# ffreyer/MonteCarlo.jl

Hardware: AMD Instinct MI355X
Metric: DQMC sweeps/sec, 16x16 Hubbard beta=8 dtau=0.1; achieved % fp64 MFMA roofline (higher is better)
Workload: dtype f64

## Files before the change

### montecarlo.jl_amd/csrc/sweep_lu.hip

```cpp
#include "kernels.h"
#include <hip/hip_ext.h>
#include <cstdlib>

namespace dqmc {

typedef double d4 __attribute__((ext_vector_type(4)));

size_t sweep_lu_image_doubles() { return LU_STRIDE; }

__device__ __forceinline__ double readlane_d(double v, int lane)
{
    const unsigned long long u = (unsigned long long)__double_as_longlong(v);
    const unsigned lo = (unsigned)__builtin_amdgcn_readlane((int)(u & 0xffffffffull), lane);
    const unsigned hi = (unsigned)__builtin_amdgcn_readlane((int)(u >> 32), lane);
    return __longlong_as_double((long long)(((unsigned long long)hi << 32) | lo));
}
#define MFMA(a, b, c) __builtin_amdgcn_mfma_f64_16x16x4f64((a), (b), (c), 0, 0, 0)
#define DQMC_GLOBAL __attribute__((address_space(1)))
typedef const DQMC_GLOBAL double *gcdp;
typedef DQMC_GLOBAL double *gdp;
typedef double d2v __attribute__((ext_vector_type(2)));
typedef const DQMC_GLOBAL d2v *gcd2p;


constexpr int LU4_SPIN = 1 << 21;
template <int NB>
struct Lu4Smem {
    double2 aST[NB][64][64];
    double xs[NB][64];
    double strip[12][NB][2][64];
    double negv[64];
    int step[64];
    int sflag[12];
    unsigned acc16[4], neg16[4];
    int ndraw[4], exh[4];
    int abort;
};
__host__ __device__ constexpr int lu4_strip_idx(int I0, int r0, int I) { return I0 == 0 ? r0 * 2 + (I - 1) : 8 + r0; }

#define LU4_ORDER() asm volatile("" ::: "memory")

__device__ __forceinline__ int lu4_wait(int *flag, int *abortf)
{
    int v = 0;
    for (int it = 0; it < LU4_SPIN; ++it) {
        v = __builtin_amdgcn_readfirstlane(__hip_atomic_load(flag, __ATOMIC_RELAXED, __HIP_MEMORY_SCOPE_WORKGROUP));
        if (v) break;
        if ((it & 63) == 63 &&
            __builtin_amdgcn_readfirstlane(__hip_atomic_load(abortf, __ATOMIC_RELAXED, __HIP_MEMORY_SCOPE_WORKGROUP)))
            return -1;
        __builtin_amdgcn_s_sleep(1);
    }
    if (!v) {
        __hip_atomic_store(abortf, 1, __ATOMIC_RELAXED, __HIP_MEMORY_SCOPE_WORKGROUP);
        return -1;
    }
    LU4_ORDER();
    return v;
}
__device__ __forceinline__ double lu4_rcp(double r)
{
    double y = __builtin_amdgcn_rcp(r);
    double e = __builtin_fma(-r, y, 1.0);
    y = __builtin_fma(y, e, y);
    e = __builtin_fma(-r, y, 1.0);
    return __builtin_fma(y, e, y);
}

extern __shared__ __attribute__((aligned(16))) double lu4_lds[];
#ifdef LU4_STAMPS
__device__ long long *lu4_stamp_ptr = nullptr;
#define LU4_STAMP(idx)                                                                       \
    do {                                                                                     \
        if ((LU4_STAMPS != 2 || (idx) >= 320) && w == 0 && (threadIdx.x & 63) == 0 && lu4_stamp_ptr)            \
            lu4_stamp_ptr[(idx)] = (long long)__builtin_amdgcn_s_memtime();                  \
    } while (0)
#else
#define LU4_STAMP(idx) do { } while (0)
#endif
#ifdef LU4_STAMPS
#ifndef FL_STAMP_BID
#define FL_STAMP_BID 1200
#endif
#define FL_STAMP(k)                                                                                    \
    do {                                                                                               \
        if (bid == FL_STAMP_BID && threadIdx.x == 0 && lu4_stamp_ptr)                                 \
            lu4_stamp_ptr[480 + (k)] = (long long)__builtin_amdgcn_s_memtime();                       \
    } while (0)
#else
#define FL_STAMP(k) do { } while (0)
#endif
template <int NB, bool FULL, bool PRO, int J>
__device__ __noinline__ void lu4_wave(int n, const double *__restrict__ Gall, long strideG, int w, int site0,
                                      int nsites, double *__restrict__ img_all, const SweepConsts &sc,
                                      unsigned long long cbits_v, double uvec, int check_sign, int site0p,
                                      const double *__restrict__ imgp_all)
{
    Lu4Smem<NB> &sm = *reinterpret_cast<Lu4Smem<NB> *>(lu4_lds);
    const int lane = threadIdx.x & 63, g = lane >> 4, ci = lane & 15;
    const unsigned long long cbits =
        ((unsigned long long)(unsigned)__builtin_amdgcn_readfirstlane((int)(cbits_v >> 32)) << 32) |
        (unsigned)__builtin_amdgcn_readfirstlane((int)(cbits_v & 0xffffffffull));
    d4 S[NB][J + 1], ST[NB][J + 1];
#pragma unroll
    for (int b = 0; b < NB; ++b) {
        const gcdp G = (gcdp)(Gall + (long)(w * NB + b) * strideG + (long)site0 * n + site0);
#pragma unroll
        for (int I = 0; I <= J; ++I)
#pragma unroll
            for (int r = 0; r < 4; ++r) {
                const int rho = 16 * I + 4 * r + g, kap = 16 * J + ci;
                if (FULL) {
                    S[b][I][r] = G[rho + (long)n * kap];
                    ST[b][I][r] = G[kap + (long)n * rho];
                } else {
                    const bool ok = rho < nsites && kap < nsites;
                    const int rc = min(rho, nsites - 1), kc = min(kap, nsites - 1);
                    const double a = G[rc + (long)n * kc], c = G[kc + (long)n * rc];
                    S[b][I][r] = ok ? a : 0.0;
                    ST[b][I][r] = ok ? c : 0.0;
                }
            }
    }
    if (PRO) {
        LU4_STAMP(400 + 8 * J + 0);
        constexpr bool EARLY = (NB == 1) && (sizeof(Lu4Smem<NB>) + LU_STRIDE * sizeof(double) <= 150 * 1024);
        double *xtra = lu4_lds + (sizeof(Lu4Smem<NB>) + 15) / 16 * 2 + LU_STRIDE;
        double *Rl = EARLY ? reinterpret_cast<double *>(&sm.aST[0][31][0]) : reinterpret_cast<double *>(&sm.aST[0][0][0]);
        double *ttx = EARLY ? xtra : Rl + 64 * 66;
        double *tt0 = xtra + 1536;
        int *pflag = reinterpret_cast<int *>(xtra + 1536 + 1024);
        const int tid = threadIdx.x;
#pragma unroll 1
        for (int b = 0; b < NB; ++b) {
            const gcdp Gin = (gcdp)(Gall + (long)(w * NB + b) * strideG);
            const gcdp imgp = (gcdp)(imgp_all + (long)(w * NB + b) * LU_STRIDE);
            const int t = site0 + 16 * J + ci;
            d4 az[4];
#pragma unroll
            for (int Jb = 0; Jb < 4; ++Jb)
#pragma unroll
                for (int r = 0; r < 4; ++r) az[Jb][r] = Gin[t + (long)n * (site0p + 16 * Jb + 4 * r + g)];
            constexpr bool STAGE = sizeof(Lu4Smem<NB>) + LU_STRIDE * sizeof(double) <= 150 * 1024;
            auto r0_col = [&](int i) { return STAGE ? (i * 256 + tid) >> 5 : tid >> 2; };
            auto r0_row = [&](int i) { return STAGE ? 2 * ((i * 256 + tid) & 31) : (tid & 3) * 16 + 2 * i; };
            d2v r0v[8];
#pragma unroll
            for (int i = 0; i < 8; ++i)
                r0v[i] = *reinterpret_cast<gcd2p>(Gin + (long)n * (site0 + r0_col(i)) + site0p + r0_row(i));
            double *imgl = lu4_lds + (sizeof(Lu4Smem<NB>) + 15) / 16 * 2;
            double opU[STAGE ? 1 : 6][4], opL[STAGE ? 1 : 6][4], opP[STAGE ? 1 : 4][4], opQ[STAGE ? 1 : 4][4], xr[4][4];
            if (STAGE) {
                constexpr int NI = (LU_STRIDE / 2 + 255) / 256;
                const gcd2p src = reinterpret_cast<gcd2p>(imgp);
                d2v *dst = reinterpret_cast<d2v *>(imgl);
                d2v iv[NI];
#pragma unroll
                for (int i = 0; i < NI; ++i) iv[i] = src[min(tid + 256 * i, LU_STRIDE / 2 - 1)];
                __builtin_amdgcn_sched_barrier(0);
#pragma unroll
                for (int i = 0; i < NI; ++i) dst[min(tid + 256 * i, LU_STRIDE / 2 - 1)] = iv[i];
            } else {
#pragma unroll
                for (int pr = 0; pr < (STAGE ? 0 : 6); ++pr)
#pragma unroll
                    for (int q = 0; q < 4; ++q) {
                        opU[pr][q] = imgp[LU_OFF_U + pr * LU_TILE + q * 64 + lane];
                        opL[pr][q] = imgp[LU_OFF_L + pr * LU_TILE + q * 64 + lane];
                    }
#pragma unroll
                for (int Jb = 0; Jb < (STAGE ? 0 : 4); ++Jb)
#pragma unroll
                    for (int q = 0; q < 4; ++q) {
                        opP[Jb][q] = imgp[LU_OFF_PT + Jb * LU_TILE + q * 64 + lane];
                        opQ[Jb][q] = imgp[LU_OFF_Q + Jb * LU_TILE + q * 64 + lane];
                    }
            }
#pragma unroll
            for (int i = 0; i < 8; ++i) *reinterpret_cast<d2v *>(Rl + r0_col(i) * 66 + r0_row(i)) = r0v[i];
            if (STAGE) __syncthreads();
#pragma unroll
            for (int Jb = 0; Jb < 4; ++Jb)
#pragma unroll
                for (int q = 0; q < 4; ++q) xr[Jb][q] = STAGE ? imgl[LU_IMG + 16 * Jb + 4 * q + g] : imgp[LU_IMG + 16 * Jb + 4 * q + g];
#define PRO_U(pr, q) (STAGE ? imgl[LU_OFF_U + (pr) * LU_TILE + (q) * 64 + lane] : opU[STAGE ? 0 : (pr)][q])
#define PRO_L(pr, q) (STAGE ? imgl[LU_OFF_L + (pr) * LU_TILE + (q) * 64 + lane] : opL[STAGE ? 0 : (pr)][q])
#define PRO_P(jb, q) (STAGE ? imgl[LU_OFF_PT + (jb) * LU_TILE + (q) * 64 + lane] : opP[STAGE ? 0 : (jb)][q])
#define PRO_Q(jb, q) (STAGE ? imgl[LU_OFF_Q + (jb) * LU_TILE + (q) * 64 + lane] : opQ[STAGE ? 0 : (jb)][q])
            d4 xz[4], tt[4];
#if defined(LU4_STAMPS) && LU4_STAMPS != 2
            LU4_STAMP(400 + 8 * J + 1);
            asm volatile("s_waitcnt vmcnt(0)" ::: "memory");
            LU4_STAMP(400 + 8 * J + 2);
#endif
#pragma unroll
            for (int Jb = 0; Jb < 4; ++Jb) {
#pragma unroll
                for (int K = 0; K < Jb; ++K)
#pragma unroll
                    for (int q = 0; q < 4; ++q) az[Jb] = MFMA(PRO_U(lu_pair(K, Jb), q), xz[K][q], az[Jb]);
                d4 z = {0.0, 0.0, 0.0, 0.0};
#pragma unroll
                for (int q = 0; q < 4; ++q) z = MFMA(PRO_P(Jb, q), az[Jb][q], z);
#pragma unroll
                for (int r = 0; r < 4; ++r) xz[Jb][r] = z[r] * xr[Jb][r];
            }
#pragma unroll
            for (int Jb = 3; Jb >= 0; --Jb) {
                d4 a = {0.0, 0.0, 0.0, 0.0};
#pragma unroll
                for (int K = Jb + 1; K < 4; ++K)
#pragma unroll
                    for (int q = 0; q < 4; ++q) a = MFMA(PRO_L(lu_pair(Jb, K), q), tt[K][q], a);
#pragma unroll
                for (int r = 0; r < 4; ++r) a[r] = xz[Jb][r] + xr[Jb][r] * a[r];
                d4 o = {0.0, 0.0, 0.0, 0.0};
#pragma unroll
                for (int q = 0; q < 4; ++q) o = MFMA(PRO_Q(Jb, q), a[q], o);
                tt[Jb] = o;
            }
#undef PRO_U
#undef PRO_L
#undef PRO_P
#undef PRO_Q
            LU4_STAMP(400 + 8 * J + 3);
            if (EARLY) {
                double *dlt = ttx;
                if (J == 0) {
#pragma unroll
                    for (int K = 0; K < 4; ++K)
#pragma unroll
                        for (int q = 0; q < 4; ++q) tt0[(K * 4 + q) * 64 + lane] = tt[K][q];
                    LU4_ORDER();
                    __hip_atomic_store(&pflag[0], 1, __ATOMIC_RELAXED, __HIP_MEMORY_SCOPE_WORKGROUP);
#pragma unroll
                    for (int K = 0; K < 4; ++K)
#pragma unroll
                        for (int q = 0; q < 4; ++q) {
                            const int sk = 16 * K + 4 * q + g;
                            ST[b][0] = MFMA(Rl[ci * 66 + sk], tt[K][q], ST[b][0]);
                            S[b][0] = MFMA(tt[K][q], Rl[ci * 66 + sk], S[b][0]);
                        }
                } else {
#pragma unroll
                    for (int K = 0; K < 4; ++K)
#pragma unroll
                        for (int q = 0; q < 4; ++q) {
                            const int sk = 16 * K + 4 * q + g;
#pragma unroll
                            for (int I = 0; I <= J; ++I) ST[b][I] = MFMA(Rl[(16 * I + ci) * 66 + sk], tt[K][q], ST[b][I]);
                            S[b][J] = MFMA(tt[K][q], Rl[(16 * J + ci) * 66 + sk], S[b][J]);
                        }
#pragma unroll
                    for (int Jc = J + 1; Jc < 4; ++Jc) {
                        d4 dl = {0.0, 0.0, 0.0, 0.0};
#pragma unroll
                        for (int K = 0; K < 4; ++K)
#pragma unroll
                            for (int q = 0; q < 4; ++q) dl = MFMA(tt[K][q], Rl[(16 * Jc + ci) * 66 + 16 * K + 4 * q + g], dl);
#pragma unroll
                        for (int r = 0; r < 4; ++r) dlt[(lu_pair(J, Jc) * 4 + r) * 64 + lane] = dl[r];
                    }
                    LU4_ORDER();
                    __hip_atomic_store(&pflag[J], 1, __ATOMIC_RELAXED, __HIP_MEMORY_SCOPE_WORKGROUP);
                    if (lu4_wait(&pflag[0], &sm.abort) > 0) {
#pragma unroll
                        for (int K = 0; K < 4; ++K)
#pragma unroll
                            for (int q = 0; q < 4; ++q)
                                S[b][0] = MFMA(tt0[(K * 4 + q) * 64 + lane], Rl[(16 * J + ci) * 66 + 16 * K + 4 * q + g], S[b][0]);
                    }
#pragma unroll
                    for (int I = 1; I < J; ++I)
                        if (lu4_wait(&pflag[I], &sm.abort) > 0) {
#pragma unroll
                            for (int r = 0; r < 4; ++r) S[b][I][r] += dlt[(lu_pair(I, J) * 4 + r) * 64 + lane];
                        }
                    LU4_ORDER();
                    __hip_atomic_store(&pflag[4 + J], 1, __ATOMIC_RELAXED, __HIP_MEMORY_SCOPE_WORKGROUP);
                }
                continue;
            }
            if (!STAGE) __syncthreads();
            LU4_STAMP(400 + 8 * J + 4);
            double *dlt = ttx;
#pragma unroll
            for (int K = 0; K < 4; ++K)
#pragma unroll
                for (int q = 0; q < 4; ++q) {
                    const int sk = 16 * K + 4 * q + g;
#pragma unroll
                    for (int I = 0; I <= J; ++I)
                        ST[b][I] = MFMA(Rl[(16 * I + ci) * 66 + sk], tt[K][q], ST[b][I]);
                    S[b][J] = MFMA(tt[K][q], Rl[(16 * J + ci) * 66 + sk], S[b][J]);
                }
#pragma unroll
            for (int Jc = J + 1; Jc < 4; ++Jc) {
                d4 dl = {0.0, 0.0, 0.0, 0.0};
#pragma unroll
                for (int K = 0; K < 4; ++K)
#pragma unroll
                    for (int q = 0; q < 4; ++q) dl = MFMA(tt[K][q], Rl[(16 * Jc + ci) * 66 + 16 * K + 4 * q + g], dl);
#pragma unroll
                for (int r = 0; r < 4; ++r) dlt[(lu_pair(J, Jc) * 4 + r) * 64 + lane] = dl[r];
            }
            __syncthreads();
#pragma unroll
            for (int I = 0; I < J; ++I)
#pragma unroll
                for (int r = 0; r < 4; ++r) S[b][I][r] += dlt[(lu_pair(I, J) * 4 + r) * 64 + lane];
            __syncthreads();
        }
        LU4_STAMP(320 + 8 * J + 7);
    }
    LU4_STAMP(320 + 8 * J + 0);
#if defined(LU4_STAMPS) && LU4_STAMPS != 2
    asm volatile("s_waitcnt vmcnt(0)" ::: "memory");
    LU4_STAMP(320 + 8 * J + 1);
#endif
    auto sgpr = [](double v) {
        const unsigned long long u = (unsigned long long)__double_as_longlong(v);
        const unsigned lo = (unsigned)__builtin_amdgcn_readfirstlane((int)(u & 0xffffffffull));
        const unsigned hi = (unsigned)__builtin_amdgcn_readfirstlane((int)(u >> 32));
        return __longlong_as_double((long long)(((unsigned long long)hi << 32) | lo));
    };
    const double g0 = sgpr(sc.gamma[0]), g1 = sgpr(sc.gamma[1]), e0 = sgpr(sc.ebos[0]), e1 = sgpr(sc.ebos[1]);
    const double du0 = sgpr(sc.dup[0]), du1 = sgpr(sc.dup[1]), dd0 = sgpr(sc.ddn[0]), dd1 = sgpr(sc.ddn[1]);
    int lastflag = 0;

#pragma unroll
    for (int I0 = 0; I0 < 4; ++I0) {
        if (!FULL && 16 * I0 >= nsites) break;
        const bool PIV = (I0 == J), HLP = (J > I0), PTQ = (J == (I0 == 0 ? 3 : (I0 == 3 ? 1 : 0)));
        if (!PIV && !HLP && !PTQ) continue;
        if (PRO && NB == 1 && J >= 2 && I0 == 1 && sizeof(Lu4Smem<NB>) + LU_STRIDE * sizeof(double) <= 150 * 1024) {
            int *pflag = reinterpret_cast<int *>(lu4_lds + (sizeof(Lu4Smem<NB>) + 15) / 16 * 2 + LU_STRIDE + 1536 + 1024);
            (void)lu4_wait(&pflag[5], &sm.abort);
            (void)lu4_wait(&pflag[6], &sm.abort);
            (void)lu4_wait(&pflag[7], &sm.abort);
        }
        d4 PT[NB], Q[NB];
        if (PTQ) {
#pragma unroll
            for (int b = 0; b < NB; ++b)
#pragma unroll
                for (int r = 0; r < 4; ++r) PT[b][r] = Q[b][r] = (4 * r + g == ci) ? 1.0 : 0.0;
        }
        int ndraw = (lastflag >> 3) & 0xfff, exhausted = (lastflag >> 2) & 1;
        unsigned accb = 0, negb = 0;
        double negv = 0.0;
        int pf_v = 0;
        double2 pf_pay[NB];
        double pf_xh[NB];
#pragma unroll
        for (int b = 0; b < NB; ++b) { pf_pay[b] = make_double2(0.0, 0.0); pf_xh[b] = 0.0; }
        double dcur[NB];
        if (PIV) {
#pragma unroll
            for (int b = 0; b < NB; ++b) dcur[b] = readlane_d(S[b][J][0], 0);
        }
#pragma unroll
        for (int r0 = 0; r0 < 4; ++r0) {
            double xv4[NB];
#pragma unroll
            for (int b = 0; b < NB; ++b) xv4[b] = 0.0;
            unsigned panel_acc = 0;
            bool stored = false;
#pragma unroll
            for (int ks = 0; ks < 4; ++ks) {
                const int c = 4 * r0 + ks, s = 16 * I0 + c;
                if (!FULL && s >= nsites) continue;
                if (PIV) {
                    LU4_STAMP(s);
                    const int spin = (int)((cbits >> s) & 1ull);
                    double det, p, xb[NB];
                    if (NB == 1) {
                        const double gamma = spin ? g1 : g0;
                        const double r = 1.0 + gamma * (1.0 - dcur[0]);
                        det = r * r;
                        p = (spin ? e1 : e0) * det;
                        xb[0] = gamma * lu4_rcp(r);
                    } else {
                        const double D0 = spin ? du1 : du0, D1 = spin ? dd1 : dd0;
                        const double R0 = 1.0 + D0 * (1.0 - dcur[0]), R1 = 1.0 + D1 * (1.0 - dcur[NB - 1]);
                        det = R0 * R1;
                        p = det;
                        const double inv_div = lu4_rcp(det);
                        xb[0] = (R1 * inv_div) * D0;
                        xb[NB - 1] = (R0 * inv_div) * D1;
                        if (check_sign && det < 0.0) {
                            negb |= 1u << c;
                            negv = lane == s ? det : negv;
                        }
                    }
                    bool acc;
                    if (p > 1.0) acc = true;
                    else {
                        const double u = readlane_d(uvec, ndraw);
                        ++ndraw;
                        if (u == 2.0) exhausted = 1;
                        acc = u < p;
                    }
                    const int word = (ndraw << 3) | (exhausted << 2);
                    const bool more = c < 15 && (FULL || s + 1 < nsites);
                    constexpr int dummy = 0;
                    (void)dummy;
                    const int c1 = c + 1, l1 = 16 * (c1 & 3) + c1;
                    {
                        const bool accu = __builtin_amdgcn_readfirstlane((int)acc) != 0;
                        accb |= (accu ? 1u : 0u) << c;
                        const bool lm2 = g == ks && ci > c;
#pragma unroll
                        for (int b = 0; b < NB; ++b) {
                            const double x = accu ? xb[b] : 0.0;
                            const double mS = lm2 ? S[b][J][r0] : 0.0, mT = lm2 ? ST[b][J][r0] : 0.0;
                            const double aS = x * mT, aT = x * mS;
                            if (more) {
                                const double qs = readlane_d(mT * mS, 16 * ks + c1);
                                dcur[b] = __builtin_fma(x, qs, readlane_d(S[b][J][c1 >> 2], l1));
                            }
                            S[b][J] = MFMA(aS, mS, S[b][J]);
                            if (c < 15) sm.aST[b][s][lane] = make_double2(aS, aT);
                            sm.xs[b][s] = x;
                            ST[b][J] = MFMA(aT, mT, ST[b][J]);
                        }
                        LU4_ORDER();
                        __hip_atomic_store(&sm.step[s], word | (accu ? 2 : 1), __ATOMIC_RELAXED, __HIP_MEMORY_SCOPE_WORKGROUP);
                    }
                    lastflag = word;
                } else {
                    if (!HLP && c == 15) continue;
                    if (HLP && J < 3 && c == 15) {
#pragma unroll
                        for (int b = 0; b < NB; ++b) {
                            sm.strip[lu4_strip_idx(I0, r0, J)][b][0][lane] = S[b][I0][r0];
                            sm.strip[lu4_strip_idx(I0, r0, J)][b][1][lane] = ST[b][I0][r0];
                        }
                        LU4_ORDER();
                        __hip_atomic_store(&sm.sflag[lu4_strip_idx(I0, r0, J)], 1, __ATOMIC_RELAXED, __HIP_MEMORY_SCOPE_WORKGROUP);
                        stored = true;
                    }
                    int v = c > 0 ? __builtin_amdgcn_readfirstlane(pf_v) : 0;
                    double2 pay[NB];
                    double xh[NB];
#pragma unroll
                    for (int b = 0; b < NB; ++b) { pay[b] = pf_pay[b]; xh[b] = pf_xh[b]; }
                    for (int it = 0; v == 0 && it < LU4_SPIN; ++it) {
                        const int vr = __hip_atomic_load(&sm.step[s], __ATOMIC_RELAXED, __HIP_MEMORY_SCOPE_WORKGROUP);
                        LU4_ORDER();
#pragma unroll
                        for (int b = 0; b < NB; ++b) {
                            if (c < 15) pay[b] = sm.aST[b][s][lane];
                            xh[b] = sm.xs[b][s];
                        }
                        v = __builtin_amdgcn_readfirstlane(vr);
                        if (v) break;
                        if ((it & 63) == 63 && __builtin_amdgcn_readfirstlane(__hip_atomic_load(
                                                   &sm.abort, __ATOMIC_RELAXED, __HIP_MEMORY_SCOPE_WORKGROUP))) {
                            v = -1;
                            break;
                        }
                        __builtin_amdgcn_s_sleep(1);
                    }
                    if (v == 0) {
                        __hip_atomic_store(&sm.abort, 1, __ATOMIC_RELAXED, __HIP_MEMORY_SCOPE_WORKGROUP);
                        v = -1;
                    }
                    if (v > 0) lastflag = v;
                    if (c < 15 && (FULL || s + 1 < nsites)) {
                        pf_v = __hip_atomic_load(&sm.step[s + 1], __ATOMIC_RELAXED, __HIP_MEMORY_SCOPE_WORKGROUP);
                        LU4_ORDER();
#pragma unroll
                        for (int b = 0; b < NB; ++b) {
                            if (c + 1 < 15) pf_pay[b] = sm.aST[b][s + 1][lane];
                            pf_xh[b] = sm.xs[b][s + 1];
                        }
                    }
                    LU4_STAMP(64 * (1 + J) + s);
                    if (v > 0 && (v & 3) == 2) {
                        panel_acc |= 1u << ks;
#pragma unroll
                        for (int b = 0; b < NB; ++b) {
                            const double aS = pay[b].x, aT = pay[b].y;
                            if (HLP) xv4[b] = g == ks ? xh[b] : xv4[b];
                            if (HLP && c < 15) {
                                S[b][I0] = MFMA(aS, S[b][I0][r0], S[b][I0]);
                                ST[b][I0] = MFMA(aT, ST[b][I0][r0], ST[b][I0]);
                            }
                            if (PTQ && c < 15) {
                                PT[b] = MFMA(aT, PT[b][r0], PT[b]);
                                Q[b] = MFMA(aS, Q[b][r0], Q[b]);
                            }
                        }
                    }
                }
            }
            if (HLP && panel_acc != 0) {
                if (J < 3 && !stored) {
#pragma unroll
                    for (int b = 0; b < NB; ++b) {
                        sm.strip[lu4_strip_idx(I0, r0, J)][b][0][lane] = S[b][I0][r0];
                        sm.strip[lu4_strip_idx(I0, r0, J)][b][1][lane] = ST[b][I0][r0];
                    }
                    LU4_ORDER();
                    __hip_atomic_store(&sm.sflag[lu4_strip_idx(I0, r0, J)], 1, __ATOMIC_RELAXED, __HIP_MEMORY_SCOPE_WORKGROUP);
                }
#pragma unroll
                for (int b = 0; b < NB; ++b) {
                    S[b][J] = MFMA(xv4[b] * ST[b][I0][r0], S[b][I0][r0], S[b][J]);
                    ST[b][J] = MFMA(xv4[b] * S[b][I0][r0], ST[b][I0][r0], ST[b][J]);
                }
#pragma unroll
                for (int I = I0 + 1; I < J; ++I) {
                    const int ok = lu4_wait(&sm.sflag[lu4_strip_idx(I0, r0, I)], &sm.abort);
                    if (ok > 0) {
#pragma unroll
                        for (int b = 0; b < NB; ++b) {
                            const double rs = sm.strip[lu4_strip_idx(I0, r0, I)][b][0][lane];
                            const double rt = sm.strip[lu4_strip_idx(I0, r0, I)][b][1][lane];
                            S[b][I] = MFMA(xv4[b] * rt, S[b][I0][r0], S[b][I]);
                            ST[b][I] = MFMA(xv4[b] * rs, ST[b][I0][r0], ST[b][I]);
                        }
                    }
                }
            }
        }
        LU4_STAMP(320 + 8 * J + 2 + I0);
#pragma unroll
        for (int b = 0; b < NB; ++b) {
            const gdp img = (gdp)(img_all + (long)(w * NB + b) * LU_STRIDE);
#pragma unroll
            for (int r = 0; r < 4; ++r) {
                const int tpos = (ci >> 2) * 64 + 16 * (ci & 3) + 4 * r + g;
                if (HLP) {
                    img[LU_OFF_U + lu_pair(I0, J) * LU_TILE + r * 64 + lane] = S[b][I0][r];
                    img[LU_OFF_L + lu_pair(I0, J) * LU_TILE + tpos] = ST[b][I0][r];
                }
                if (PTQ) {
                    img[LU_OFF_PT + I0 * LU_TILE + tpos] = PT[b][r];
                    img[LU_OFF_Q + I0 * LU_TILE + r * 64 + lane] = Q[b][r];
                }
            }
            if (PIV && (lane >> 4) == I0) img[LU_IMG + lane] = sm.xs[b][lane];
        }
        if (PIV) {
            if (lane == 0) {
                sm.acc16[I0] = accb;
                sm.neg16[I0] = negb;
                sm.ndraw[I0] = ndraw;
                sm.exh[I0] = exhausted;
            }
            if (NB == 2 && (lane >> 4) == I0) sm.negv[lane] = negv;
        }
    }
    LU4_STAMP(320 + 8 * J + 6);
}

template <int NB, bool FULL, bool PRO>
__device__ __forceinline__ void lu4_block(int w, int n, const double *__restrict__ Gall, long strideG,
                                          int8_t *__restrict__ conf_slice, long conf_stride, int site0, int nsites,
                                          double *__restrict__ img_all, const SweepConsts &sc, WalkerRng *rngs,
                                          DevStats *stats, int check_sign, int *errflag, int site0p,
                                          const double *__restrict__ imgp_all)
{
    Lu4Smem<NB> &sm = *reinterpret_cast<Lu4Smem<NB> *>(lu4_lds);
    const int tid = threadIdx.x, lane = tid & 63, wave = tid >> 6;
    int8_t *__restrict__ cw = conf_slice + (long)w * conf_stride;
    const int myc = (FULL || lane < nsites) ? (int)cw[site0 + (FULL ? lane : min(lane, nsites - 1))] : 1;
    const unsigned long long cbits = __ballot(myc > 0);
    const WalkerRng rs = rngs[w];
    double uvec;
    {
        const unsigned long long d = rs.draw + (unsigned long long)lane;
        uvec = rs.uniforms ? (d < rs.n_uniforms ? rs.uniforms[d] : 2.0) : philox_uniform(rs.seed, d);
    }
    if (tid < 64) {
        sm.step[tid] = 0;
        for (int b = 0; b < NB; ++b) sm.xs[b][tid] = 0.0;
    }
    if (tid < 12) sm.sflag[tid] = 0;
#ifdef LU4_STAMPS
    if (w == 0 && tid == 0 && lu4_stamp_ptr) lu4_stamp_ptr[360] = (long long)__builtin_amdgcn_s_memtime();
#endif
    if (tid < 4) { sm.acc16[tid] = 0u; sm.neg16[tid] = 0u; sm.ndraw[tid] = 0; sm.exh[tid] = 0; }
    if (tid == 0) sm.abort = 0;
    if (PRO && NB == 1 && tid < 8)
        reinterpret_cast<int *>(lu4_lds + (sizeof(Lu4Smem<NB>) + 15) / 16 * 2 + LU_STRIDE + 1536 + 1024)[tid] = 0;
    __syncthreads();
    const int wv = __builtin_amdgcn_readfirstlane(wave);
    if (wv == 0) lu4_wave<NB, FULL, PRO, 0>(n, Gall, strideG, w, site0, nsites, img_all, sc, cbits, uvec, check_sign, site0p, imgp_all);
    else if (wv == 1) lu4_wave<NB, FULL, PRO, 1>(n, Gall, strideG, w, site0, nsites, img_all, sc, cbits, uvec, check_sign, site0p, imgp_all);
    else if (wv == 2) lu4_wave<NB, FULL, PRO, 2>(n, Gall, strideG, w, site0, nsites, img_all, sc, cbits, uvec, check_sign, site0p, imgp_all);
    else lu4_wave<NB, FULL, PRO, 3>(n, Gall, strideG, w, site0, nsites, img_all, sc, cbits, uvec, check_sign, site0p, imgp_all);
    __syncthreads();
    const int nblk = (nsites + 15) / 16;
    if (!FULL) {
        const int I0 = wv, g = lane >> 4, ci = lane & 15;
        if (I0 >= nblk)
            for (int b = 0; b < NB; ++b) {
                const gdp img = (gdp)(img_all + (long)(w * NB + b) * LU_STRIDE);
                for (int r = 0; r < 4; ++r) {
                    const double idv = (4 * r + g == ci) ? 1.0 : 0.0;
                    for (int Jc = I0 + 1; Jc < 4; ++Jc) {
                        img[LU_OFF_U + lu_pair(I0, Jc) * LU_TILE + r * 64 + lane] = 0.0;
                        img[LU_OFF_L + lu_pair(I0, Jc) * LU_TILE + r * 64 + lane] = 0.0;
                    }
                    img[LU_OFF_PT + I0 * LU_TILE + r * 64 + lane] = idv;
                    img[LU_OFF_Q + I0 * LU_TILE + r * 64 + lane] = idv;
                }
                if (lane < 16) img[LU_IMG + 16 * I0 + lane] = 0.0;
            }
    }
    if (wv == 0) {
        const unsigned long long accbits = (unsigned long long)sm.acc16[0] | ((unsigned long long)sm.acc16[1] << 16) |
                                           ((unsigned long long)sm.acc16[2] << 32) | ((unsigned long long)sm.acc16[3] << 48);
        if (lane < nsites && ((accbits >> lane) & 1ull)) cw[site0 + lane] = (int8_t)(-myc);
        if (lane == 0) {
            rngs[w].draw = rs.draw + (unsigned long long)sm.ndraw[nblk - 1];
            if (sm.exh[nblk - 1]) rngs[w].exhausted = 1;
            stats[w].prop_local += nsites;
            stats[w].acc_local += __popcll(accbits);
            if (sm.abort) atomicOr(errflag, 2);
#ifdef LU4_STAMPS
            if (w == 0 && lu4_stamp_ptr) lu4_stamp_ptr[361] = (long long)__builtin_amdgcn_s_memtime();
#endif
            if (NB == 2)
                for (int s = 0; s < nsites; ++s)
                    if ((sm.neg16[s >> 4] >> (s & 15)) & 1u) magstats_push(stats[w].negative_probability, sm.negv[s]);
        }
    }
}

template <int NB, bool FULL>
__global__ __launch_bounds__(256) void sweep_lu4_kernel(int n, const double *__restrict__ Gall, long strideG,
                                                       int8_t *__restrict__ conf_slice, long conf_stride, int site0,
                                                       int nsites, double *__restrict__ img_all, SweepConsts sc,
                                                       WalkerRng *rngs, DevStats *stats, int check_sign, int *errflag)
{
    lu4_block<NB, FULL, false>(blockIdx.x, n, Gall, strideG, conf_slice, conf_stride, site0, nsites, img_all, sc, rngs,
                               stats, check_sign, errflag, 0, nullptr);
}

hipError_t launch_sweep_lu(int n, int nb, int n_walkers, const double *G, long strideG, int8_t *conf_slice,
                           long conf_stride, int site0, int nsites, double *img, SweepConsts sc, WalkerRng *rng,
                           DevStats *stats, int check_sign, int *errflag, hipStream_t s, hipEvent_t start,
                           hipEvent_t stop)
{
    if (nsites < 1 || nsites > 64 || site0 < 0 || site0 + nsites > n || nb < 1 || nb > 2) return hipErrorInvalidValue;
    const bool full = nsites == 64;
    int dev = 0;
    (void)hipGetDevice(&dev);
    static unsigned attr_mask = 0;
    if (!(attr_mask & (1u << dev))) {
        (void)hipFuncSetAttribute((const void *)sweep_lu4_kernel<1, true>, hipFuncAttributeMaxDynamicSharedMemorySize, (int)sizeof(Lu4Smem<1>));
        (void)hipFuncSetAttribute((const void *)sweep_lu4_kernel<1, false>, hipFuncAttributeMaxDynamicSharedMemorySize, (int)sizeof(Lu4Smem<1>));
        (void)hipFuncSetAttribute((const void *)sweep_lu4_kernel<2, true>, hipFuncAttributeMaxDynamicSharedMemorySize, (int)sizeof(Lu4Smem<2>));
        (void)hipFuncSetAttribute((const void *)sweep_lu4_kernel<2, false>, hipFuncAttributeMaxDynamicSharedMemorySize, (int)sizeof(Lu4Smem<2>));
        attr_mask |= 1u << dev;
    }
    dim3 grid(n_walkers), block(256);
#define LU4_LAUNCH(NBV, FL)                                                                                          \
    hipExtLaunchKernelGGL((sweep_lu4_kernel<NBV, FL>), grid, block, sizeof(Lu4Smem<NBV>), s, start, stop, 0, n, G, strideG, \
                          conf_slice, conf_stride, site0, nsites, img, sc, rng, stats, check_sign, errflag)
    if (nb == 1) { if (full) LU4_LAUNCH(1, true); else LU4_LAUNCH(1, false); }
    else { if (full) LU4_LAUNCH(2, true); else LU4_LAUNCH(2, false); }
#undef LU4_LAUNCH
    return hipGetLastError();
}

constexpr int FL_LDR = 66;
template <bool FULL, int NT, int NCP = 1>
__device__ __forceinline__ void flush_lu_body(int bid, int n, int n_units, const double *__restrict__ Gin_all,
                                              double *__restrict__ Gout_all, long strideG, int site0, int nsites,
                                              const double *__restrict__ img_all, int tiles_m, int tiles_n,
                                              int ncp_rt = 1)
{
    const int ncp = NCP > 0 ? NCP : ncp_rt;
    double *fsm = lu4_lds;
    double *img = fsm;
    double *xs = fsm + LU_IMG;
    double *Rl = fsm + LU_STRIDE;
    const int xcd = bid & 7, seq = bid >> 3;
    const int T = tiles_m * tiles_n;
    const int unit = (seq / T) * 8 + xcd;
    if (unit >= n_units) return;
    const int tile = seq % T;
    const int m0 = (tile % tiles_m) * 64, n00 = (tile / tiles_m) * (16 * NT * ncp);
    int n0 = n00;
    const gcdp Gin = (gcdp)(Gin_all + (long)unit * strideG);
    const gdp Gout = (gdp)(Gout_all + (long)unit * strideG);
    const int tid = threadIdx.x, lane = tid & 63, wave = tid >> 6, g = lane >> 4, ci = lane & 15;
    const int t = m0 + 16 * wave + ci;
    const int tq = FULL ? t : min(t, n - 1);

    FL_STAMP(0);
    d4 acc[NT];
#pragma unroll
    for (int jt = 0; jt < NT; ++jt)
#pragma unroll
        for (int r = 0; r < 4; ++r) {
            const int tp = n0 + 16 * jt + 4 * r + g;
            acc[jt][r] = Gin[tq + (long)n * (FULL ? tp : min(tp, n - 1))];
        }
    d4 az[4];
#pragma unroll
    for (int J = 0; J < 4; ++J)
#pragma unroll
        for (int r = 0; r < 4; ++r) {
            const int s = 16 * J + 4 * r + g;
            const int col = site0 + (FULL ? s : min(s, nsites - 1));
            double v = Gin[tq + (long)n * col];
            if (!FULL && (s >= nsites || t >= n)) v = 0.0;
            az[J][r] = v - ((t == site0 + s) ? 1.0 : 0.0);
        }
    {
        const gcd2p src = reinterpret_cast<gcd2p>((gcdp)(img_all + (long)unit * LU_STRIDE));
        d2v *dst = reinterpret_cast<d2v *>(img);
        for (int i = tid; i < LU_STRIDE / 2; i += 256) dst[i] = src[i];
    }
#pragma unroll
    for (int pass = 0; pass < NT / 4; ++pass) {
        const int tl = pass * 64 + (tid >> 2), tp = n0 + tl, s0 = (tid & 3) * 16;
        double *d = Rl + tl * FL_LDR + s0;
        if (FULL) {
            d2v rv[8];
#pragma unroll
            for (int i = 0; i < 8; ++i) {
                const int pc = i * 256 + tid, col = pass * 64 + (pc >> 5), w2 = 2 * (pc & 31);
                rv[i] = *reinterpret_cast<gcd2p>(Gin + (long)n * (n0 + col) + site0 + w2);
            }
#pragma unroll
            for (int i = 0; i < 8; ++i) {
                const int pc = i * 256 + tid, col = pass * 64 + (pc >> 5), w2 = 2 * (pc & 31);
                *reinterpret_cast<d2v *>(Rl + col * FL_LDR + w2) = rv[i];
            }
        } else {
            for (int i = 0; i < 16; ++i)
                d[i] = (tp < n && s0 + i < nsites) ? Gin[(long)n * tp + site0 + s0 + i] : 0.0;
        }
    }
    __syncthreads();
    FL_STAMP(1);

    d4 xz[4];
#pragma unroll
    for (int J = 0; J < 4; ++J) {
#pragma unroll
        for (int K = 0; K < J; ++K)
#pragma unroll
            for (int q = 0; q < 4; ++q)
                az[J] = MFMA(img[LU_OFF_U + lu_pair(K, J) * LU_TILE + q * 64 + lane], xz[K][q], az[J]);
        d4 z = {0.0, 0.0, 0.0, 0.0};
#pragma unroll
        for (int q = 0; q < 4; ++q) z = MFMA(img[LU_OFF_PT + J * LU_TILE + q * 64 + lane], az[J][q], z);
#pragma unroll
        for (int r = 0; r < 4; ++r) xz[J][r] = z[r] * xs[16 * J + 4 * r + g];
    }
    d4 tt[4];
#pragma unroll
    for (int J = 3; J >= 0; --J) {
        d4 a = {0.0, 0.0, 0.0, 0.0};
#pragma unroll
        for (int K = J + 1; K < 4; ++K)
#pragma unroll
            for (int q = 0; q < 4; ++q)
                a = MFMA(img[LU_OFF_L + lu_pair(J, K) * LU_TILE + q * 64 + lane], tt[K][q], a);
#pragma unroll
        for (int r = 0; r < 4; ++r) a[r] = xz[J][r] + xs[16 * J + 4 * r + g] * a[r];
        d4 o = {0.0, 0.0, 0.0, 0.0};
#pragma unroll
        for (int q = 0; q < 4; ++q) o = MFMA(img[LU_OFF_Q + J * LU_TILE + q * 64 + lane], a[q], o);
        tt[J] = o;
    }
    if constexpr (NCP == 0 && FULL && NT == 4) {
        const int rb_off[2] = {(int)(Rl - fsm), 0};
        FL_STAMP(2);
        __syncthreads();
        FL_STAMP(3);
        for (int cp = 0; cp < ncp; ++cp) {
            const bool more = cp + 1 < ncp;
            const int n1 = n00 + (more ? cp + 1 : cp) * 64;
            d4 nxt[NT];
            double r0n[16];
#pragma unroll
            for (int jt = 0; jt < NT; ++jt)
#pragma unroll
                for (int r = 0; r < 4; ++r) nxt[jt][r] = Gin[t + (long)n * (n1 + 16 * jt + 4 * r + g)];
#pragma unroll
            for (int i = 0; i < 8; ++i) {
                const int pc = i * 256 + tid;
                const d2v v = *reinterpret_cast<gcd2p>(Gin + (long)n * (n1 + (pc >> 5)) + site0 + 2 * (pc & 31));
                r0n[2 * i] = v.x;
                r0n[2 * i + 1] = v.y;
            }
            const double *Rc = fsm + rb_off[cp & 1];
#pragma unroll
            for (int K = 0; K < 4; ++K)
#pragma unroll
                for (int q = 0; q < 4; ++q) {
                    const int sk = 16 * K + 4 * q + g;
#pragma unroll
                    for (int jt = 0; jt < NT; ++jt) acc[jt] = MFMA(Rc[(16 * jt + ci) * FL_LDR + sk], tt[K][q], acc[jt]);
                }
            n0 = n00 + cp * 64;
#pragma unroll
            for (int jt = 0; jt < NT; ++jt)
#pragma unroll
                for (int r = 0; r < 4; ++r) Gout[t + (long)n * (n0 + 16 * jt + 4 * r + g)] = acc[jt][r];
            if (more) {
                double *nb = fsm + rb_off[(cp + 1) & 1];
#pragma unroll
                for (int i = 0; i < 8; ++i) {
                    const int pc = i * 256 + tid;
                    *reinterpret_cast<double2 *>(nb + (pc >> 5) * FL_LDR + 2 * (pc & 31)) = make_double2(r0n[2 * i], r0n[2 * i + 1]);
                }
#pragma unroll
                for (int jt = 0; jt < NT; ++jt) acc[jt] = nxt[jt];
                __syncthreads();
            }
            FL_STAMP(4 + cp);
        }
        return;
    }
    for (int cp = 0; cp < ncp; ++cp) {
        if (cp > 0) {
            n0 = n00 + cp * 16 * NT;
#pragma unroll
            for (int jt = 0; jt < NT; ++jt)
#pragma unroll
                for (int r = 0; r < 4; ++r) {
                    const int tp = n0 + 16 * jt + 4 * r + g;
                    acc[jt][r] = Gin[tq + (long)n * (FULL ? tp : min(tp, n - 1))];
                }
            __syncthreads();
#pragma unroll
            for (int pass = 0; pass < NT / 4; ++pass) {
                const int tl = pass * 64 + (tid >> 2), tp = n0 + tl, s0 = (tid & 3) * 16;
                double *d = Rl + tl * FL_LDR + s0;
                if (FULL) {
                    d2v rv[8];
#pragma unroll
                    for (int i = 0; i < 8; ++i) {
                        const int pc = i * 256 + tid, col = pass * 64 + (pc >> 5), w2 = 2 * (pc & 31);
                        rv[i] = *reinterpret_cast<gcd2p>(Gin + (long)n * (n0 + col) + site0 + w2);
                    }
#pragma unroll
                    for (int i = 0; i < 8; ++i) {
                        const int pc = i * 256 + tid, col = pass * 64 + (pc >> 5), w2 = 2 * (pc & 31);
                        *reinterpret_cast<d2v *>(Rl + col * FL_LDR + w2) = rv[i];
                    }
                } else {
                    for (int i = 0; i < 16; ++i)
                        d[i] = (tp < n && s0 + i < nsites) ? Gin[(long)n * tp + site0 + s0 + i] : 0.0;
                }
            }
            __syncthreads();
        }
#pragma unroll
        for (int K = 0; K < 4; ++K)
#pragma unroll
            for (int q = 0; q < 4; ++q) {
                const int sk = 16 * K + 4 * q + g;
#pragma unroll
                for (int jt = 0; jt < NT; ++jt)
                    acc[jt] = MFMA(Rl[(16 * jt + ci) * FL_LDR + sk], tt[K][q], acc[jt]);
            }
#pragma unroll
        for (int jt = 0; jt < NT; ++jt)
#pragma unroll
            for (int r = 0; r < 4; ++r) {
                const int tp = n0 + 16 * jt + 4 * r + g;
                if (FULL || (t < n && tp < n)) Gout[t + (long)n * tp] = acc[jt][r];
            }
    }
}

template <bool FULL, int NT, int NCP = 1>
__global__ __launch_bounds__(256) void sweep_flush_lu_kernel(int n, int n_units, const double *__restrict__ Gin_all,
                                                            double *__restrict__ Gout_all, long strideG, int site0,
                                                            int nsites, const double *__restrict__ img_all,
                                                            int tiles_m, int tiles_n, int ncp_rt)
{
    flush_lu_body<FULL, NT, NCP>(blockIdx.x, n, n_units, Gin_all, Gout_all, strideG, site0, nsites, img_all, tiles_m, tiles_n,
                                 ncp_rt);
}

struct SweepFusedArgs {
    int n, n_walkers, n_units;
    const double *Gin;
    double *Gout;
    long strideG;
    int8_t *conf_slice;
    long conf_stride;
    int site0, site0p;
    double *img;
    const double *imgp;
    SweepConsts sc;
    WalkerRng *rngs;
    DevStats *stats;
    int check_sign;
    int *errflag;
    int tiles_m, tiles_n;
};
template <int NB, int NT, int NCP>
__global__ __launch_bounds__(256) void sweep_fused_kernel(SweepFusedArgs a)
{
    if ((int)blockIdx.x < a.n_walkers)
        lu4_block<NB, true, true>(blockIdx.x, a.n, a.Gin, a.strideG, a.conf_slice, a.conf_stride, a.site0, 64, a.img, a.sc,
                                  a.rngs, a.stats, a.check_sign, a.errflag, a.site0p, a.imgp);
    else
        flush_lu_body<true, NT, NCP>((int)blockIdx.x - a.n_walkers, a.n, a.n_units, a.Gin, a.Gout, a.strideG, a.site0p, 64,
                                     a.imgp, a.tiles_m, a.tiles_n);
}


hipError_t launch_sweep_flush_lu(int n, int n_units, const double *Gin, double *Gout, long strideG, int site0,
                                 int nsites, const double *img, const KernelSwitches &sw, hipStream_t s, hipEvent_t start,
                                 hipEvent_t stop)
{
    const bool wide = n % 128 == 0;
    const int nt = wide ? 8 : 4;
    const int tm = (n + 63) / 64, tn = (n + 16 * nt - 1) / (16 * nt);
    const int groups = (n_units + 7) / 8;
    const size_t lds = ((size_t)LU_STRIDE + 16 * nt * FL_LDR) * sizeof(double);
    const bool full = (n % 64 == 0) && nsites == 64;
    int dev = 0;
    (void)hipGetDevice(&dev);
    static unsigned attr_mask = 0;
    if (!(attr_mask & (1u << dev))) {
        const int big = (int)(((size_t)LU_STRIDE + 128 * FL_LDR) * sizeof(double));
        (void)hipFuncSetAttribute((const void *)sweep_flush_lu_kernel<true, 8>, hipFuncAttributeMaxDynamicSharedMemorySize, big);
        (void)hipFuncSetAttribute((const void *)sweep_flush_lu_kernel<false, 8>, hipFuncAttributeMaxDynamicSharedMemorySize, big);
        (void)hipFuncSetAttribute((const void *)sweep_flush_lu_kernel<true, 4>, hipFuncAttributeMaxDynamicSharedMemorySize, big);
        (void)hipFuncSetAttribute((const void *)sweep_flush_lu_kernel<false, 4>, hipFuncAttributeMaxDynamicSharedMemorySize, big);
        attr_mask |= 1u << dev;
    }
#define FL_LAUNCH(FU, NTV)                                                                                          \
    hipExtLaunchKernelGGL((sweep_flush_lu_kernel<FU, NTV>), dim3(groups * 8 * tm * tn), dim3(256), lds, s, start, stop, 0, \
                          n, n_units, Gin, Gout, strideG, site0, nsites, img, tm, tn, 1)
    static int n_cus[32] = {0};
    if (dev >= 0 && dev < 32 && n_cus[dev] == 0) {
        hipDeviceProp_t prop;
        n_cus[dev] = hipGetDeviceProperties(&prop, dev) == hipSuccess ? prop.multiProcessorCount : 256;
    }
    const bool ncp2 = sw.flush_ncp2 || (dev >= 0 && dev < 32 && groups * 8 * tm * tn > n_cus[dev]);
    if (ncp2 && full && (n + 63) / 64 > 1) {
        const int tn4 = (n + 63) / 64;
        const size_t lds4 = ((size_t)LU_STRIDE + 64 * FL_LDR) * sizeof(double);
        static unsigned m0 = 0;
        if (!(m0 & (1u << dev))) {
            (void)hipFuncSetAttribute((const void *)sweep_flush_lu_kernel<true, 4, 0>, hipFuncAttributeMaxDynamicSharedMemorySize,
                                      (int)(((size_t)LU_STRIDE + 128 * FL_LDR) * sizeof(double)));
            m0 |= 1u << dev;
        }
        hipExtLaunchKernelGGL((sweep_flush_lu_kernel<true, 4, 0>), dim3(groups * 8 * tm), dim3(256), lds4, s, start, stop, 0, n,
                              n_units, Gin, Gout, strideG, site0, nsites, img, tm, 1, tn4);
        return hipGetLastError();
    }
    if (wide) { if (full) FL_LAUNCH(true, 8); else FL_LAUNCH(false, 8); }
    else { if (full) FL_LAUNCH(true, 4); else FL_LAUNCH(false, 4); }
#undef FL_LAUNCH
    return hipGetLastError();
}

hipError_t launch_sweep_fused(int n, int nb, int n_walkers, const double *Gin, double *Gout, long strideG,
                              int8_t *conf_slice, long conf_stride, int site0, int site0p, double *img,
                              const double *imgp, SweepConsts sc, WalkerRng *rng, DevStats *stats, int check_sign,
                              int *errflag, hipStream_t s, hipEvent_t start, hipEvent_t stop)
{
    if (n % 64 != 0 || site0 % 64 != 0 || site0p % 64 != 0 || site0 + 64 > n || site0p + 64 > n || nb < 1 || nb > 2)
        return hipErrorInvalidValue;
    const int n_units = n_walkers * nb;
    const bool wide = n % 128 == 0;
    const int nt = wide ? 8 : 4;
    SweepFusedArgs a;
    a.n = n; a.n_walkers = n_walkers; a.n_units = n_units; a.Gin = Gin; a.Gout = Gout; a.strideG = strideG;
    a.conf_slice = conf_slice; a.conf_stride = conf_stride; a.site0 = site0; a.site0p = site0p; a.img = img; a.imgp = imgp;
    a.sc = sc; a.rngs = rng; a.stats = stats; a.check_sign = check_sign; a.errflag = errflag;
    const int ncp = (wide && n % 256 == 0) ? 2 : 1;
    a.tiles_m = n / 64; a.tiles_n = n / (16 * nt * ncp);
    const int groups = (n_units + 7) / 8;
    const int flush_blocks = groups * 8 * a.tiles_m * a.tiles_n;
    const size_t lds_flush = ((size_t)LU_STRIDE + 16 * nt * FL_LDR) * sizeof(double);
    const size_t lds_lu = nb == 1 ? sizeof(Lu4Smem<1>) : sizeof(Lu4Smem<2>);
    const size_t lds_pro = nb == 1 ? (sizeof(Lu4Smem<1>) + 15) / 16 * 16 + (LU_STRIDE + 1536 + 1024 + 8) * sizeof(double) : lds_lu;
    const size_t lds_e = lds_pro > lds_lu ? lds_pro : lds_lu;
    const size_t lds = lds_flush > lds_e ? lds_flush : lds_e;
    int dev = 0;
    (void)hipGetDevice(&dev);
    static unsigned attr_mask = 0;
    if (!(attr_mask & (1u << dev))) {
        (void)hipFuncSetAttribute((const void *)sweep_fused_kernel<1, 8, 1>, hipFuncAttributeMaxDynamicSharedMemorySize, 160 * 1024);
        (void)hipFuncSetAttribute((const void *)sweep_fused_kernel<1, 8, 2>, hipFuncAttributeMaxDynamicSharedMemorySize, 160 * 1024);
        (void)hipFuncSetAttribute((const void *)sweep_fused_kernel<1, 4, 1>, hipFuncAttributeMaxDynamicSharedMemorySize, 160 * 1024);
        (void)hipFuncSetAttribute((const void *)sweep_fused_kernel<2, 8, 1>, hipFuncAttributeMaxDynamicSharedMemorySize, 160 * 1024);
        (void)hipFuncSetAttribute((const void *)sweep_fused_kernel<2, 8, 2>, hipFuncAttributeMaxDynamicSharedMemorySize, 160 * 1024);
        (void)hipFuncSetAttribute((const void *)sweep_fused_kernel<2, 4, 1>, hipFuncAttributeMaxDynamicSharedMemorySize, 160 * 1024);
        attr_mask |= 1u << dev;
    }
    dim3 grid(n_walkers + flush_blocks), block(256);
#define FU_LAUNCH(NBV, NTV, NCPV) hipExtLaunchKernelGGL((sweep_fused_kernel<NBV, NTV, NCPV>), grid, block, lds, s, start, stop, 0, a)
    if (nb == 1) { if (ncp == 2) FU_LAUNCH(1, 8, 2); else if (wide) FU_LAUNCH(1, 8, 1); else FU_LAUNCH(1, 4, 1); }
    else { if (ncp == 2) FU_LAUNCH(2, 8, 2); else if (wide) FU_LAUNCH(2, 8, 1); else FU_LAUNCH(2, 4, 1); }
#undef FU_LAUNCH
    return hipGetLastError();
}

#ifdef LU4_STAMPS
extern "C" int dqmc_debug_lu4_stamps(void *devptr)
{
    return (int)hipMemcpyToSymbol(HIP_SYMBOL(lu4_stamp_ptr), &devptr, sizeof(void *));
}
#endif

}
```

Measured before the change: 812.1.

## Move config/RNG head setup into one helper wave and share via LDS flag

The per-block prologue that read the spin configuration, built the sign ballot and drew the uniform random numbers (philox or table lookup) ran on every wave before the LU waves started. That work now runs on a single designated wave (wave 3 for the early-prologue path, wave 0 otherwise), overlapped with its prologue. The results go into new LDS fields guarded by a flag, and the other waves fetch them just before they are needed. This takes global loads and RNG work off the critical path at kernel start. In exchange it adds LDS footprint, a spin-wait on the flag, and ordering that depends on relaxed atomics and compiler barriers.

```diff
diff --git a/montecarlo.jl_amd/csrc/sweep_lu.hip b/montecarlo.jl_amd/csrc/sweep_lu.hip
--- a/montecarlo.jl_amd/csrc/sweep_lu.hip
+++ b/montecarlo.jl_amd/csrc/sweep_lu.hip
@@ -35,7 +35,13 @@
     unsigned acc16[4], neg16[4];
     int ndraw[4], exh[4];
     int abort;
+    double huvec[64];
+    unsigned long long hcbits;
+    unsigned long long hdraw;
+    int hmyc[64];
+    int hflag;
 };
+static_assert(sizeof(Lu4Smem<2>) <= 160 * 1024, "the two-block elimination has to fit a CU's LDS");
 __host__ __device__ constexpr int lu4_strip_idx(int I0, int r0, int I) { return I0 == 0 ? r0 * 2 + (I - 1) : 8 + r0; }
 
 #define LU4_ORDER() asm volatile("" ::: "memory")
@@ -93,14 +99,15 @@
 template <int NB, bool FULL, bool PRO, int J>
 __device__ __noinline__ void lu4_wave(int n, const double *__restrict__ Gall, long strideG, int w, int site0,
                                       int nsites, double *__restrict__ img_all, const SweepConsts &sc,
-                                      unsigned long long cbits_v, double uvec, int check_sign, int site0p,
-                                      const double *__restrict__ imgp_all)
+                                      const int8_t *__restrict__ cw, const WalkerRng *__restrict__ rng, int check_sign,
+                                      int site0p, const double *__restrict__ imgp_all)
 {
     Lu4Smem<NB> &sm = *reinterpret_cast<Lu4Smem<NB> *>(lu4_lds);
     const int lane = threadIdx.x & 63, g = lane >> 4, ci = lane & 15;
-    const unsigned long long cbits =
-        ((unsigned long long)(unsigned)__builtin_amdgcn_readfirstlane((int)(cbits_v >> 32)) << 32) |
-        (unsigned)__builtin_amdgcn_readfirstlane((int)(cbits_v & 0xffffffffull));
+    constexpr bool EARLY = PRO && (NB == 1) && (sizeof(Lu4Smem<NB>) + LU_STRIDE * sizeof(double) <= 150 * 1024);
+    constexpr int HW = EARLY ? 3 : 0;
+    unsigned long long cbits = 0ull;
+    double uvec = 0.0;
     d4 S[NB][J + 1], ST[NB][J + 1];
 #pragma unroll
     for (int b = 0; b < NB; ++b) {
@@ -122,9 +129,49 @@
                 }
             }
     }
+    int h_myc = 1;
+    unsigned long long h_seed = 0ull, h_draw = 0ull, h_nuni = 0ull;
+    gcdp h_uni = nullptr;
+    if (J == HW) {
+        h_myc = ((const DQMC_GLOBAL int8_t *)cw)[site0 + (FULL ? lane : min(lane, nsites - 1))];
+        const DQMC_GLOBAL WalkerRng *rg = (const DQMC_GLOBAL WalkerRng *)rng;
+        h_seed = rg->seed;
+        h_draw = rg->draw;
+        h_uni = (gcdp)rg->uniforms;
+        h_nuni = rg->n_uniforms;
+    }
+    auto sgpr64 = [](unsigned long long u) {
+        return ((unsigned long long)(unsigned)__builtin_amdgcn_readfirstlane((int)(u >> 32)) << 32) |
+               (unsigned)__builtin_amdgcn_readfirstlane((int)(u & 0xffffffffull));
+    };
+    auto head_deposit = [&]() {
+        const int myc = (FULL || lane < nsites) ? h_myc : 1;
+        const unsigned long long cb = __ballot(myc > 0);
+        const unsigned long long draw = sgpr64(h_draw), nuni = sgpr64(h_nuni);
+        const gcdp uni = (gcdp)sgpr64((unsigned long long)h_uni);
+        const unsigned long long d = draw + (unsigned long long)lane;
+        const double u = uni ? (d < nuni ? uni[d] : 2.0) : philox_uniform(sgpr64(h_seed), d);
+        sm.huvec[lane] = u;
+        sm.hmyc[lane] = myc;
+        if (lane == 0) {
+            sm.hcbits = cb;
+            sm.hdraw = draw;
+        }
+        LU4_ORDER();
+        __hip_atomic_store(&sm.hflag, 1, __ATOMIC_RELAXED, __HIP_MEMORY_SCOPE_WORKGROUP);
+        if (!PRO) {
+            cbits = cb;
+            uvec = u;
+        }
+    };
+    auto head_fetch = [&]() {
+        LU4_ORDER();
+        uvec = sm.huvec[lane];
+        cbits = sgpr64(sm.hcbits);
+    };
+    if (!PRO && J == HW) head_deposit();
     if (PRO) {
         LU4_STAMP(400 + 8 * J + 0);
-        constexpr bool EARLY = (NB == 1) && (sizeof(Lu4Smem<NB>) + LU_STRIDE * sizeof(double) <= 150 * 1024);
         double *xtra = lu4_lds + (sizeof(Lu4Smem<NB>) + 15) / 16 * 2 + LU_STRIDE;
         double *Rl = EARLY ? reinterpret_cast<double *>(&sm.aST[0][31][0]) : reinterpret_cast<double *>(&sm.aST[0][0][0]);
         double *ttx = EARLY ? xtra : Rl + 64 * 66;
@@ -179,6 +226,7 @@
 #pragma unroll
             for (int i = 0; i < 8; ++i) *reinterpret_cast<d2v *>(Rl + r0_col(i) * 66 + r0_row(i)) = r0v[i];
             if (STAGE) __syncthreads();
+            if (J == HW && b == 0) head_deposit();
 #pragma unroll
             for (int Jb = 0; Jb < 4; ++Jb)
 #pragma unroll
@@ -233,6 +281,8 @@
                         for (int q = 0; q < 4; ++q) tt0[(K * 4 + q) * 64 + lane] = tt[K][q];
                     LU4_ORDER();
                     __hip_atomic_store(&pflag[0], 1, __ATOMIC_RELAXED, __HIP_MEMORY_SCOPE_WORKGROUP);
+                    (void)lu4_wait(&sm.hflag, &sm.abort);
+                    head_fetch();
 #pragma unroll
                     for (int K = 0; K < 4; ++K)
 #pragma unroll
@@ -312,6 +362,7 @@
             __syncthreads();
         }
         LU4_STAMP(320 + 8 * J + 7);
+        if (!EARLY && J == 0) head_fetch();
     }
     LU4_STAMP(320 + 8 * J + 0);
 #if defined(LU4_STAMPS) && LU4_STAMPS != 2
@@ -467,6 +518,7 @@
                         v = -1;
                     }
                     if (v > 0) lastflag = v;
+                    if (HLP && I0 == J - 1 && c == 0) head_fetch();
                     if (c < 15 && (FULL || s + 1 < nsites)) {
                         pf_v = __hip_atomic_load(&sm.step[s + 1], __ATOMIC_RELAXED, __HIP_MEMORY_SCOPE_WORKGROUP);
                         LU4_ORDER();
@@ -566,14 +618,6 @@
     Lu4Smem<NB> &sm = *reinterpret_cast<Lu4Smem<NB> *>(lu4_lds);
     const int tid = threadIdx.x, lane = tid & 63, wave = tid >> 6;
     int8_t *__restrict__ cw = conf_slice + (long)w * conf_stride;
-    const int myc = (FULL || lane < nsites) ? (int)cw[site0 + (FULL ? lane : min(lane, nsites - 1))] : 1;
-    const unsigned long long cbits = __ballot(myc > 0);
-    const WalkerRng rs = rngs[w];
-    double uvec;
-    {
-        const unsigned long long d = rs.draw + (unsigned long long)lane;
-        uvec = rs.uniforms ? (d < rs.n_uniforms ? rs.uniforms[d] : 2.0) : philox_uniform(rs.seed, d);
-    }
     if (tid < 64) {
         sm.step[tid] = 0;
         for (int b = 0; b < NB; ++b) sm.xs[b][tid] = 0.0;
@@ -583,15 +627,15 @@
     if (w == 0 && tid == 0 && lu4_stamp_ptr) lu4_stamp_ptr[360] = (long long)__builtin_amdgcn_s_memtime();
 #endif
     if (tid < 4) { sm.acc16[tid] = 0u; sm.neg16[tid] = 0u; sm.ndraw[tid] = 0; sm.exh[tid] = 0; }
-    if (tid == 0) sm.abort = 0;
+    if (tid == 0) { sm.abort = 0; sm.hflag = 0; }
     if (PRO && NB == 1 && tid < 8)
         reinterpret_cast<int *>(lu4_lds + (sizeof(Lu4Smem<NB>) + 15) / 16 * 2 + LU_STRIDE + 1536 + 1024)[tid] = 0;
     __syncthreads();
     const int wv = __builtin_amdgcn_readfirstlane(wave);
-    if (wv == 0) lu4_wave<NB, FULL, PRO, 0>(n, Gall, strideG, w, site0, nsites, img_all, sc, cbits, uvec, check_sign, site0p, imgp_all);
-    else if (wv == 1) lu4_wave<NB, FULL, PRO, 1>(n, Gall, strideG, w, site0, nsites, img_all, sc, cbits, uvec, check_sign, site0p, imgp_all);
-    else if (wv == 2) lu4_wave<NB, FULL, PRO, 2>(n, Gall, strideG, w, site0, nsites, img_all, sc, cbits, uvec, check_sign, site0p, imgp_all);
-    else lu4_wave<NB, FULL, PRO, 3>(n, Gall, strideG, w, site0, nsites, img_all, sc, cbits, uvec, check_sign, site0p, imgp_all);
+    if (wv == 0) lu4_wave<NB, FULL, PRO, 0>(n, Gall, strideG, w, site0, nsites, img_all, sc, cw, rngs + w, check_sign, site0p, imgp_all);
+    else if (wv == 1) lu4_wave<NB, FULL, PRO, 1>(n, Gall, strideG, w, site0, nsites, img_all, sc, cw, rngs + w, check_sign, site0p, imgp_all);
+    else if (wv == 2) lu4_wave<NB, FULL, PRO, 2>(n, Gall, strideG, w, site0, nsites, img_all, sc, cw, rngs + w, check_sign, site0p, imgp_all);
+    else lu4_wave<NB, FULL, PRO, 3>(n, Gall, strideG, w, site0, nsites, img_all, sc, cw, rngs + w, check_sign, site0p, imgp_all);
     __syncthreads();
     const int nblk = (nsites + 15) / 16;
     if (!FULL) {
@@ -614,9 +658,9 @@
     if (wv == 0) {
         const unsigned long long accbits = (unsigned long long)sm.acc16[0] | ((unsigned long long)sm.acc16[1] << 16) |
                                            ((unsigned long long)sm.acc16[2] << 32) | ((unsigned long long)sm.acc16[3] << 48);
-        if (lane < nsites && ((accbits >> lane) & 1ull)) cw[site0 + lane] = (int8_t)(-myc);
+        if (lane < nsites && ((accbits >> lane) & 1ull)) cw[site0 + lane] = (int8_t)(-sm.hmyc[lane]);
         if (lane == 0) {
-            rngs[w].draw = rs.draw + (unsigned long long)sm.ndraw[nblk - 1];
+            rngs[w].draw = sm.hdraw + (unsigned long long)sm.ndraw[nblk - 1];
             if (sm.exh[nblk - 1]) rngs[w].exhausted = 1;
             stats[w].prop_local += nsites;
             stats[w].acc_local += __popcll(accbits);
```

Result: no change. 812.0 (-0.0%).
